# mika314/melonix

Hardware: AMD Instinct MI355X
Metric: STFT+pitch+resynth frames/sec (48 kHz, 4096 FFT, 256 hop); % HBM roofline (higher is better)
Workload: dtype f32

## Files before the change

melonix_amd/csrc/resynth_kernels.hip:

```cpp
#include <hip/hip_runtime.h>

#include "kernels.h"

#pragma clang fp contract(off)

namespace mx {

namespace {

constexpr int kResynthThreads = 128;

__global__ __launch_bounds__(kResynthThreads) void resynth_kernel(const ResynthArgs a) {
  const mx_step st = a.steps[blockIdx.x];
  const float *g = a.audio + MX_AUDIO_PAD + st.grain_start;
  const int L = st.grain_len;
  const float rate = st.rate;
  const float next = st.next_first;
  float *of = a.pcm_f32 ? a.pcm_f32 + st.out_offset : nullptr;
  int16_t *oi = a.pcm_i16 ? a.pcm_i16 + st.out_offset : nullptr;
  for (int i = threadIdx.x; i < st.sz; i += kResynthThreads) {
    const float x = (float)i * rate;
    const float ip = __builtin_truncf(x);
    const float f = x - ip;
    const int idx = (int)ip;
    const float a0 = g[idx];
    const float a1 = (idx + 1 < L) ? g[idx + 1] : next;
    const float v = (1.f - f) * a0 + f * a1;
    if (of) of[i] = v;
    if (oi) oi[i] = (int16_t)((double)v * 32767.);
  }
}

constexpr int kMaxGrain = 2304;

__device__ __forceinline__ float lerp_tap(const float *lg, int i, float rate) {
  const float x = (float)i * rate;
  const float ip = __builtin_truncf(x);
  const float f = x - ip;
  const int idx = (int)ip;
  return (1.f - f) * lg[idx] + f * lg[idx + 1];
}

__global__ __launch_bounds__(kResynthThreads) void resynth_kernel_v(const ResynthArgs a) {
  __shared__ __attribute__((aligned(16))) float lds[kMaxGrain + 8];
  const mx_step st = a.steps[blockIdx.x];
  const int L = st.grain_len, sz = st.sz, tid = threadIdx.x;
  const float *g = a.audio + MX_AUDIO_PAD + st.grain_start;
  if (L > kMaxGrain) {
    float *of = a.pcm_f32 ? a.pcm_f32 + st.out_offset : nullptr;
    int16_t *oi = a.pcm_i16 ? a.pcm_i16 + st.out_offset : nullptr;
    for (int i = tid; i < sz; i += kResynthThreads) {
      const float x = (float)i * st.rate;
      const float ip = __builtin_truncf(x);
      const float f = x - ip;
      const int idx = (int)ip;
      const float a1 = (idx + 1 < L) ? g[idx + 1] : st.next_first;
      const float v = (1.f - f) * g[idx] + f * a1;
      if (of) of[i] = v;
      if (oi) oi[i] = (int16_t)((double)v * 32767.);
    }
    return;
  }
  const int shift = (int)((reinterpret_cast<uintptr_t>(g) >> 2) & 3);
  const float4 *ga = reinterpret_cast<const float4 *>(g - shift);
  float4 *l4 = reinterpret_cast<float4 *>(lds);
  for (int j = tid; j < (L + shift + 4) / 4; j += kResynthThreads) l4[j] = ga[j];
  __syncthreads();
  float *lg = lds + shift;
  if (tid == 0) lg[L] = st.next_first;
  __syncthreads();

  float *of = a.pcm_f32 ? a.pcm_f32 + st.out_offset : nullptr;
  int16_t *oi = a.pcm_i16 ? a.pcm_i16 + st.out_offset : nullptr;
  const float rate = st.rate;
  const int head = (int)((8 - (st.out_offset & 7)) & 7) < sz ? (int)((8 - (st.out_offset & 7)) & 7) : sz;
  const int nv = (sz - head) / 8;
  for (int q = tid; q < nv; q += kResynthThreads) {
    const int i0 = head + 8 * q;
    float v[8];
#pragma unroll
    for (int k = 0; k < 8; ++k) v[k] = lerp_tap(lg, i0 + k, rate);
    if (of) {
      float4 *o4 = reinterpret_cast<float4 *>(of + i0);
      o4[0] = make_float4(v[0], v[1], v[2], v[3]);
      o4[1] = make_float4(v[4], v[5], v[6], v[7]);
    }
    if (oi) {
      unsigned w[4];
#pragma unroll
      for (int k = 0; k < 4; ++k) {
        const unsigned lo = (unsigned)(unsigned short)(int16_t)((double)v[2 * k] * 32767.);
        const unsigned hi = (unsigned)(unsigned short)(int16_t)((double)v[2 * k + 1] * 32767.);
        w[k] = lo | (hi << 16);
      }
      *reinterpret_cast<uint4 *>(oi + i0) = make_uint4(w[0], w[1], w[2], w[3]);
    }
  }
  const int tail0 = head + 8 * nv;
  for (int i = tid; i < head + (sz - tail0); i += kResynthThreads) {
    const int ii = i < head ? i : tail0 + (i - head);
    const float v = lerp_tap(lg, ii, rate);
    if (of) of[ii] = v;
    if (oi) oi[ii] = (int16_t)((double)v * 32767.);
  }
}

__device__ __forceinline__ uint64_t bit_range(int64_t base, int64_t lo, int64_t hi) {
  const int64_t s = lo - base > 0 ? lo - base : 0;
  const int64_t e = hi - base < 64 ? hi - base : 64;
  if (e <= s) return 0ull;
  const uint64_t upto_e = e >= 64 ? ~0ull : ((1ull << e) - 1ull);
  return upto_e & ~((1ull << s) - 1ull);
}

__global__ __launch_bounds__(256) void zc_kernel(const float *__restrict__ wav ,
                                                 int64_t n, uint64_t *__restrict__ zc7,
                                                 uint64_t *__restrict__ zc3) {
  const int lane = threadIdx.x & 63;
  const int64_t w0 = ((int64_t)blockIdx.x * 4 + (threadIdx.x >> 6)) * 64;
  const int64_t nwords = (n + 63) >> 6;
  if (w0 >= nwords) return;
  const float *p = wav + w0 * 64 + lane;
  const float xp = p[-64], xn = p[64 * 64];
  const uint64_t Aprev = __ballot(!(xp >= 0.f)), Bnext = __ballot(!(xn < 0.f));
  uint64_t A = 0, B = 0;
#pragma unroll 16
  for (int w = 0; w < 64; ++w) {
    const float x = p[64 * w];
    const uint64_t a = __ballot(!(x >= 0.f)), b = __ballot(!(x < 0.f));
    if (lane == w) {
      A = a;
      B = b;
    }
  }
  uint64_t Ap = ((uint64_t)(unsigned)__shfl_up((int)(A >> 32), 1) << 32) | (unsigned)__shfl_up((int)A, 1);
  uint64_t Bn = ((uint64_t)(unsigned)__shfl_down((int)(B >> 32), 1) << 32) | (unsigned)__shfl_down((int)B, 1);
  if (lane == 0) Ap = Aprev;
  if (lane == 63) Bn = Bnext;
  uint64_t ra3 = A, ra7 = A, rb3 = ~0ull, rb7 = ~0ull;
#pragma unroll
  for (int j = 1; j <= 7; ++j) {
    const uint64_t bj = (B >> j) | (Bn << (64 - j));
    rb7 &= bj;
    if (j <= 3) rb3 &= bj;
    if (j <= 6) {
      const uint64_t aj = (A << j) | (Ap >> (64 - j));
      ra7 &= aj;
      if (j <= 2) ra3 &= aj;
    }
  }
  const int64_t wi = w0 + lane;
  if (wi < nwords) {
    zc7[wi] = ra7 & rb7 & bit_range(wi * 64, 7, n - 7 - 1);
    zc3[wi] = ra3 & rb3 & bit_range(wi * 64, 3, n - 3 - 1);
  }
}

__global__ __launch_bounds__(256) void resynth_tail_kernel(const ResynthArgs a) {
  const mx_step last = a.steps[a.nsteps - 1];
  const int64_t covered = last.out_offset + (int64_t)last.sz;
  for (int64_t i = covered + (int64_t)blockIdx.x * 256 + threadIdx.x; i < a.nsamples; i += (int64_t)gridDim.x * 256) {
    if (a.pcm_f32) a.pcm_f32[i] = 0.f;
    if (a.pcm_i16) a.pcm_i16[i] = 0;
  }
}

}

hipError_t launch_resynth(const ResynthArgs &a, hipStream_t s) {
  if (a.nsteps > 0x7fffffffLL) return hipErrorInvalidValue;
  if (a.nsteps > 0) {
    hipLaunchKernelGGL(resynth_tail_kernel, dim3(64), dim3(256), 0, s, a);
    const bool aligned = ((reinterpret_cast<uintptr_t>(a.pcm_f32) | reinterpret_cast<uintptr_t>(a.pcm_i16) |
                           reinterpret_cast<uintptr_t>(a.audio)) & 15) == 0;
    if (aligned) {
      hipLaunchKernelGGL(resynth_kernel_v, dim3((unsigned)a.nsteps), dim3(kResynthThreads), 0, s, a);
    } else {
      hipLaunchKernelGGL(resynth_kernel, dim3((unsigned)a.nsteps), dim3(kResynthThreads), 0, s, a);
    }
    hipError_t e = hipGetLastError();
    if (e != hipSuccess) return e;
  }
  return hipSuccess;
}

hipError_t launch_zc_bitmaps(const float *audio_padded, int64_t n, uint64_t *zc7, uint64_t *zc3,
                             hipStream_t s) {
  if (n <= 0) return hipSuccess;
  const int64_t blocks = (((n + 63) >> 6) + 255) / 256;
  if (blocks > 0x7fffffffLL) return hipErrorInvalidValue;
  static_assert(MX_AUDIO_PAD >= 64 * 65, "zc_kernel reads one block row past either end of the audio");
  hipLaunchKernelGGL(zc_kernel, dim3((unsigned)blocks), dim3(256), 0, s, audio_padded + MX_AUDIO_PAD, n,
                     zc7, zc3);
  return hipGetLastError();
}

}
```

melonix_amd/csrc/stft_kernel_impl.h:

```cpp
#pragma once
#include <hip/hip_runtime.h>

#include "colormap_core.h"
#include "kernels.h"
#include "stft_core.h"
#include "stft_tables.h"

#define MX_BARRIER() __syncthreads()

namespace mx {

template <bool MAXOP>
__device__ __forceinline__ unsigned wave_reduce_u32(unsigned k) {
  constexpr unsigned ident = MAXOP ? 0u : 0xffffffffu;
#define MX_DPP_STEP(CTRL, ROWS)                                                                      \
  {                                                                                                  \
    const unsigned o = (unsigned)__builtin_amdgcn_update_dpp((int)ident, (int)k, CTRL, ROWS, 0xf, false); \
    k = MAXOP ? (o > k ? o : k) : (o < k ? o : k);                                                   \
  }
  MX_DPP_STEP(0xB1, 0xf)
  MX_DPP_STEP(0x4E, 0xf)
  MX_DPP_STEP(0x141, 0xf)
  MX_DPP_STEP(0x140, 0xf)
  MX_DPP_STEP(0x142, 0xa)
  MX_DPP_STEP(0x143, 0xc)
#undef MX_DPP_STEP
  return (unsigned)__builtin_amdgcn_readlane((int)k, 63);
}
__device__ __forceinline__ unsigned long long wave_max_u64(unsigned long long k) {
  const unsigned hi = (unsigned)(k >> 32), lo = (unsigned)k;
  const unsigned mhi = wave_reduce_u32<true>(hi);
  const unsigned long long tie = __ballot(hi == mhi);
  unsigned mlo;
  if (__builtin_popcountll(tie) == 1) mlo = (unsigned)__builtin_amdgcn_readlane((int)lo, __builtin_ctzll(tie));
  else mlo = wave_reduce_u32<true>(hi == mhi ? lo : 0u);
  return ((unsigned long long)mhi << 32) | mlo;
}

template <int IMM, bool NT = true>
__device__ __forceinline__ void st_row_nt(const float *base, unsigned off, float x) {
  static_assert(IMM >= -4096 && IMM <= 4095, "global_store immediate offset");
#if defined(__HIP_DEVICE_COMPILE__)
  if constexpr (NT) asm volatile("global_store_dword %0, %1, %2 offset:%3 nt" : : "v"(off), "v"(x), "s"(base), "n"(IMM) : "memory");
  else asm volatile("global_store_dword %0, %1, %2 offset:%3" : : "v"(off), "v"(x), "s"(base), "n"(IMM) : "memory");
#endif
}

template <class P, int MODE, int HOP, int WPE, bool DEFER = false, bool PREFETCH = false, bool CMAP = false, bool DIRECT = false,
          bool CIRC = false>
__global__ __launch_bounds__(P::T) __attribute__((amdgpu_waves_per_eu(WPE, WPE)))
void stft_kernel(const StftArgs a0) {
  const StftArgs &a = a0;
  using C = P;
  constexpr int N = P::N;
  constexpr int NW = C::T / 64;
  constexpr int kRed = (NW > 1) ? ((NW + 1) / 2) * 2 : 0;
  constexpr bool kTw3Bases = (P::R3 == 16);
  constexpr int kTw2 = ((C::TW2 + 1) / 2) * 2;
  static_assert(P::R3 == 16 || P::R3 == 8, "twiddle placement per plan");
  static_assert(!DIRECT || (NW > 1 && !DEFER && !CMAP), "direct row stores: multi-wave, non-deferred plans");
  static_assert(!CIRC || (MODE != kRanges && HOP == 0 && !PREFETCH && !CMAP), "circular window: bulk modes");
  constexpr int IMG = t1_size<C>();
  __shared__ __attribute__((aligned(16))) float2 lds[IMG + kRed + (DEFER ? C::M / 2 : 0) + kTw2];
  float *const lout = reinterpret_cast<float *>(DEFER ? lds + IMG + kRed : lds);
  float2 *const ltw2 = lds + IMG + kRed + (DEFER ? C::M / 2 : 0);

  const int t_ = threadIdx.x;
  const bool wave0 = __builtin_amdgcn_readfirstlane(t_) < 64;
  cpx u[kTw3Bases ? 1 : P::R3];
  cpx ulo;
  cpx w3r[kTw3Bases ? 1 : P::R3 - 1], w3base[6];
  if constexpr (kTw3Bases) {
    cpx uhi_unused;
    post_bases<P>(t_, a.ubase, ulo, uhi_unused);
    fetch_tw3_bases<P>(t_, a.tw3, w3base);
  } else {
    post_twiddles<P>(t_, a.ubase, *reinterpret_cast<cpx(*)[P::R3]>(&u));
    fetch_tw3<P>(t_, a.tw3, *reinterpret_cast<cpx(*)[P::R3 - 1]>(&w3r));
  }
  const uint32_t bmask_ = band_mask<P>(t_, a.kmin, a.kmax);
  uint32_t umask = 0;
#pragma unroll
  for (int o = 0; o < P::E; ++o) umask |= (__ballot((bmask_ >> o) & 1u) != 0ull) ? (1u << o) : 0u;
  umask = __builtin_amdgcn_readfirstlane(umask);
  constexpr bool kSlide = (MODE == kBulkAligned) && (HOP > 0) && Slide<P, (HOP > 0 ? HOP : 2)>::ok;
  constexpr int SD = Slide<P, (HOP > 0 ? HOP : 2)>::D;
  constexpr float kSc = 0.5f / (float)N;
  for (int i = t_; i < C::TW2; i += C::T) ltw2[i] = a.tw2[i];
  MX_BARRIER();

  unsigned lb = blockIdx.x;
  {
    const unsigned nb = gridDim.x, xcd = lb & 7u, q = nb >> 3, r = nb & 7u;
    lb = (xcd < r ? xcd * (q + 1) : r * (q + 1) + (xcd - r) * q) + (lb >> 3);
  }
  const int64_t f0 = (int64_t)lb * a.frames_per_block;
  const int64_t f1 = (f0 + a.frames_per_block < a.count) ? f0 + a.frames_per_block : a.count;

  cpx Y[P::E];
  cpx edge[SD], nx[SD];
  if constexpr (kSlide) {
    const int64_t e0 = (a.first_frame + f0 + 1) * (int64_t)HOP;
    if (f0 < f1) load_frame<P, 1, true>(t_, Y, a.audio + MX_AUDIO_PAD + (e0 - N), a.wtab);
    slide_edge<P, HOP>(t_, a.wtab, 2.0f * (float)N, edge);
  }

  unsigned long long *const red = reinterpret_cast<unsigned long long *>(lds + IMG);
  auto flush_pitch = [&](int64_t fr, int tt) {
    if (a.pitch && tt == 0) {
      unsigned long long b = red[0];
#pragma unroll
      for (int i = 1; i < NW; ++i) b = red[i] > b ? red[i] : b;
      mx_pitch p;
      p.bin = 0x7fffffff - (int)(unsigned)(b & 0xffffffffull);
      p.mag = __uint_as_float((unsigned)(b >> 32));
      a.pitch[fr] = p;
    }
  };
  const bool want_rows = a.mags != nullptr || (CMAP && a.rgb != nullptr);
  auto flush_row = [&](int64_t fr, int tt) {
    if (want_rows) {
      using f32x4 = float __attribute__((ext_vector_type(4)));
      const f32x4 *l4 = reinterpret_cast<const f32x4 *>(lout) + tt;
      f32x4 *row4 = reinterpret_cast<f32x4 *>(a.mags + (size_t)fr * (size_t)(N / 2)) + tt;
      f32x4 q[C::M / 4 / C::T];
#pragma unroll
      for (int i = 0; i < C::M / 4 / C::T; ++i) q[i] = l4[C::T * i];
      if (!CMAP || a.mags) {
#pragma unroll
        for (int i = 0; i < C::M / 4 / C::T; ++i) {
          __builtin_nontemporal_store(q[i], &row4[C::T * i]);
        }
      }
      if constexpr (CMAP) {
        if (a.rgb) {
          uint32_t *trow = reinterpret_cast<uint32_t *>(a.rgb + (size_t)fr * (size_t)(N / 2) * 3) + 3 * tt;
#pragma unroll 1
          for (int i = 0; i < C::M / 4 / C::T; ++i) {
            uint32_t w3[3];
            texel4(q[i].x, q[i].y, q[i].z, q[i].w, a.cmap_k, w3);
            uint32_t *o = trow + 3 * C::T * i;
            o[0] = w3[0];
            o[1] = w3[1];
            o[2] = w3[2];
          }
        }
      }
    }
  };

  auto frame_ptrs = [&](int64_t fr, int zo, const float *&x, const float *&w) {
    if constexpr (MODE == kRanges) {
      const int s = a.ranges[2 * fr], e = a.ranges[2 * fr + 1];
      const bool outside = (e <= 0) || ((int64_t)e - N >= a.n);
      x = outside ? a.audio : a.audio + MX_AUDIO_PAD + ((int64_t)e - N);
      int64_t d0 = (int64_t)N - ((int64_t)e - (int64_t)s);
      d0 = d0 < (int64_t)(N - 1 - kWOff) ? (int64_t)(N - 1 - kWOff) : d0;
      d0 = d0 > (int64_t)(kWDmax + kWTail) ? (int64_t)(kWDmax + kWTail) : d0;
      w = a.wext + kWOff + d0;
    } else {
      const int64_t e = (a.first_frame + fr + 1) * (int64_t)a.hop;
      x = a.audio + MX_AUDIO_PAD + (e - N);
      w = a.wtab + zo;
    }
  };
  float cpx_[2 * Circ<P>::CS], cpw_[2 * Circ<P>::CS];
  if constexpr (CIRC) {
    if (f0 < f1) {
      const int64_t pe = (a.first_frame + f0 + 1) * (int64_t)a.hop;
      circ_load_first<P>(t_, Y, a.audio + MX_AUDIO_PAD + (pe - N), a.wtab, circ_geo<P>(pe, a.hop).o);
    }
  }
  cpx xr[(PREFETCH && !kSlide) ? P::E : 1];
  if constexpr (PREFETCH && !kSlide) {
    if (f0 < f1) {
      const float *x0;
      const float *w0;
      frame_ptrs(f0, 0, x0, w0);
      load_raw<P, (MODE == kBulkAligned)>(t_, xr, x0);
    }
  }

  for (int64_t f = f0; f < f1; ++f) {
    int t = t_;
    unsigned bmask = bmask_;
    int zoff = 0;
    asm volatile("" : "+v"(t), "+v"(bmask), "+s"(zoff));
    int out_lo, out_hi;
    out_bases<P>(t, out_lo, out_hi);

    if constexpr (CIRC) {
      if (f > f0) {
        const int64_t pe = (a.first_frame + f + 1) * (int64_t)a.hop;
        const CircGeo<P> geo = circ_geo<P>(pe, a.hop);
        circ_fetch<P>(t, a.audio + MX_AUDIO_PAD + (pe - 2 * (int64_t)a.hop), a.wtab + zoff + (N - 2 * a.hop), geo, cpx_, cpw_);
        circ_step<P>(t, Y, a.decay, geo, cpx_, cpw_);
      }
    } else if constexpr (kSlide) {
      if (f > f0) slide_step<P, HOP>(Y, nx, edge, a.decay, kSc);
      if (f + 1 < f1) slide_fetch<P, HOP>(t, a.audio + MX_AUDIO_PAD + (a.first_frame + f + 2) * (int64_t)HOP, nx);
    } else {
      const float *x;
      const float *w;
      frame_ptrs(f, zoff, x, w);
      if constexpr (PREFETCH) {
        if constexpr (MODE == kRanges) apply_window<P, -1, false>(t, Y, xr, w);
        else apply_window_geo<P>(t, Y, xr, a.wtab + N + zoff, a.hop);
      } else if constexpr (MODE == kRanges) {
        load_frame<P, -1, false>(t, Y, x, w);
      } else {
        load_frame_geo<P, (MODE == kBulkAligned)>(t, Y, x, a.wtab + N + zoff, a.hop);
      }
    }

    cpx v[P::E];
    pass1<P>(Y, v);
    constexpr bool kTw2Batch = (P::NB2 == 1);
    store_t1<P>(t, v, lds);
    MX_BARRIER();
    if constexpr (DEFER || DIRECT) {
      if (f > f0) flush_pitch(f - 1, t);
    }
    if constexpr (kTw2Batch) {
      cpx w2[P::R2 - 1];
      load_t1_tw2<P>(t, v, lds, ltw2, w2);
      if constexpr (DEFER) {
        if (f > f0) flush_row(f - 1, t);
      }
      MX_BARRIER();
      pass2_reg<P>(v, w2);
    } else {
      load_t1<P>(t, v, lds);
      if constexpr (DEFER) {
        if (f > f0) flush_row(f - 1, t);
      }
      MX_BARRIER();
      pass2<P>(t, v, ltw2);
    }
    store_t2<P>(t, v, lds);
    MX_BARRIER();
    load_t2<P>(t, v, lds);
    MX_BARRIER();
    float mg[P::E];
    if (NW == 1 || wave0) {
      if constexpr (kTw3Bases) {
        pass3_bases<P, true>(t, v, w3base);
        post_fly<P, true>(t, v, ulo, csel(t == 0, mk(-1.0f, 0.0f), ulo), mg);
      } else {
        pass3_reg<P, true>(t, v, *reinterpret_cast<cpx(*)[P::R3 - 1]>(&w3r));
        post<P, true>(t, v, *reinterpret_cast<cpx(*)[P::R3]>(&u), mg);
      }
    } else {
      if constexpr (kTw3Bases) {
        pass3_bases<P, false>(t, v, w3base);
        post_fly<P, false>(t, v, ulo, ulo, mg);
      } else {
        pass3_reg<P, false>(t, v, *reinterpret_cast<cpx(*)[P::R3 - 1]>(&w3r));
        post<P, false>(t, v, *reinterpret_cast<cpx(*)[P::R3]>(&u), mg);
      }
    }

    if constexpr (PREFETCH && !kSlide) {
      if (f + 1 < f1) {
        const float *xn;
        const float *wn;
        frame_ptrs(f + 1, zoff, xn, wn);
        load_raw<P, (MODE == kBulkAligned)>(t, xr, xn);
      }
    }

    unsigned long long best = 0ull;
    if (a.pitch) {
      const unsigned klo = 0x7fffffffu - (unsigned)out_lo, khi = 0x7fffffffu - (unsigned)out_hi;
      const unsigned nlo = 0x7fffffffu - (unsigned)(C::M - out_lo), nhi = 0x7fffffffu - (unsigned)(C::M - out_hi);
#pragma unroll
      for (int s = 0; s < C::R3; ++s) {
        constexpr int H = C::R3 / 2;
        if (!((umask >> (2 * s)) & 3u)) continue;
        const unsigned b0 = (s < H ? klo : khi) - (unsigned)(C::NS3 * s);
        unsigned b1 = (s < H ? nlo : nhi) + (unsigned)(C::NS3 * s);
        if (s == H) b1 = (t == 0) ? 0x7fffffffu - (unsigned)(C::M / 2) : b1;
        const unsigned v0 = (unsigned)((int)(bmask << (31 - 2 * s)) >> 31);
        const unsigned v1 = (unsigned)((int)(bmask << (31 - (2 * s + 1))) >> 31);
        const unsigned long long k0 = ((unsigned long long)(__float_as_uint(mg[2 * s]) & v0) << 32) | (b0 & v0);
        const unsigned long long k1 = ((unsigned long long)(__float_as_uint(mg[2 * s + 1]) & v1) << 32) | (b1 & v1);
        best = k0 > best ? k0 : best;
        best = k1 > best ? k1 : best;
      }
      best = wave_max_u64(best);
      if constexpr (NW > 1) {
        if ((t & 63) == 0) red[t >> 6] = best;
      }
    }

    if constexpr (DIRECT) {
      if (want_rows) {
        const float *row = a.mags + (size_t)f * (size_t)(N / 2);
        constexpr int H = C::R3 / 2;
        constexpr int STEP = 4 * C::NS3;
        constexpr int G = 8192 / STEP;
        static_assert((STEP == 4096 || STEP == 2048) && H % G == 0, "slot groups share an offset through the store's immediate");
        const unsigned blo = 4u * (unsigned)out_lo, bhi = 4u * (unsigned)(out_hi + C::NS3 * H);
        const unsigned nlo = 4u * (unsigned)(C::M - out_lo), nhi = 4u * (unsigned)(C::M - out_hi - C::NS3 * H);
        static_for<0, C::R3>([&](auto ss) {
          constexpr int s = decltype(ss)::value;
          constexpr int sl = s < H ? s : s - H;
          constexpr int su = (sl & ~(G - 1)) + G / 2, sd = (sl & ~(G - 1)) + G / 2 - 1;
          const unsigned o0 = (s < H ? blo : bhi) + (unsigned)(su * STEP);
          unsigned o1 = (s < H ? nlo : nhi) - (unsigned)(sd * STEP);
          if constexpr (s == H) {
            o1 = (t == 0) ? (unsigned)(4 * (C::M / 2)) + (unsigned)((sl - sd) * STEP) : o1;
          }
          st_row_nt<(sl - su) * STEP>(row, o0, mg[2 * s]);
          st_row_nt<-(sl - sd) * STEP, false>(row, o1, mg[2 * s + 1]);
        });
      }
    } else if (want_rows) {
      float *plo = lout + out_lo, *phi = lout + out_hi;
      float *mlo = lout + (C::M - out_lo), *mhi = lout + (C::M - out_hi);
#pragma unroll
      for (int s = 0; s < C::R3; ++s) {
        constexpr int H = C::R3 / 2;
        (s < H ? plo : phi)[C::NS3 * s] = mg[2 * s];
        if (s == H) (t == 0 ? lout + C::M / 2 : mhi - C::NS3 * H)[0] = mg[2 * s + 1];
        else (s < H ? mlo : mhi)[-C::NS3 * s] = mg[2 * s + 1];
      }
    }
    if constexpr (!DEFER && !DIRECT) {
      if (want_rows) {
        MX_BARRIER();
        flush_row(f, t);
        MX_BARRIER();
      } else {
        MX_BARRIER();
      }
      if constexpr (NW > 1) {
        flush_pitch(f, t);
      } else if (a.pitch && t == 0) {
        mx_pitch p;
        p.bin = 0x7fffffff - (int)(unsigned)(best & 0xffffffffull);
        p.mag = __uint_as_float((unsigned)(best >> 32));
        a.pitch[f] = p;
      }
    }
  }
  if constexpr (DEFER || DIRECT) {
    if (f0 < f1) {
      MX_BARRIER();
      flush_pitch(f1 - 1, t_);
      if constexpr (DEFER) flush_row(f1 - 1, t_);
    }
  }
}


}
```

melonix_amd/csrc/stft_kernels.hip:

```cpp
#include <hip/hip_runtime.h>

#include "kernels.h"
#include "stft_kernel_impl.h"

namespace mx {

namespace {

template <class P>
struct Tune {
  static constexpr bool TWO_WAVE = (P::E == 16);
  static constexpr int WPE = TWO_WAVE ? 3 : 2;
  static constexpr bool PREFETCH = (P::E == 32);
  static constexpr bool slides(int hop) {
    return P::N == 4096 ? (hop == 256 || hop == 512) : P::N == 16384 ? (hop == 512 || hop == 1024) : hop == 1024;
  }
  static constexpr bool DIRECT = (P::N >= 16384);
  static constexpr bool CIRC = (P::N >= 16384);
  static constexpr bool DEFER = TWO_WAVE;
};

template <class P, int HOP>
bool try_slide(const StftArgs &b, dim3 grid, dim3 block, hipStream_t s) {
  if constexpr (Slide<P, HOP>::ok && Tune<P>::slides(HOP)) {
    if (b.hop != HOP) return false;
    hipLaunchKernelGGL((stft_kernel<P, kBulkAligned, HOP, Tune<P>::WPE, Tune<P>::DEFER, false, false, Tune<P>::DIRECT>),
                       grid, block, 0, s, b);
    return true;
  } else {
    return false;
  }
}

template <class P>
bool try_circ(const StftArgs &b, dim3 grid, dim3 block, hipStream_t s) {
  if constexpr (!Tune<P>::CIRC) {
    return false;
  } else {
    if (!Circ<P>::ok(b.hop)) return false;
    hipLaunchKernelGGL((stft_kernel<P, kBulkAny, 0, Tune<P>::WPE, Tune<P>::DEFER, false, false, Tune<P>::DIRECT, true>),
                       grid, block, 0, s, b);
    return true;
  }
}

template <class P>
hipError_t launch_plan(int mode, const StftArgs &a, hipStream_t s) {
  if (a.count <= 0) return hipSuccess;
  const int g = a.frames_per_block > 0 ? a.frames_per_block : 1;
  const int64_t blocks = (a.count + g - 1) / g;
  if (blocks > 0x7fffffffLL) return hipErrorInvalidValue;
  StftArgs b = a;
  b.frames_per_block = g;
  const dim3 grid((unsigned)blocks), block(P::T);
  constexpr int W = Tune<P>::WPE;
  constexpr bool DF = Tune<P>::DEFER, PF = Tune<P>::PREFETCH, DR = Tune<P>::DIRECT;
  switch (mode) {
    case kBulkAligned:
      if (!(try_slide<P, 256>(b, grid, block, s) || try_slide<P, 512>(b, grid, block, s) ||
            try_slide<P, 1024>(b, grid, block, s) || try_circ<P>(b, grid, block, s)))
        hipLaunchKernelGGL((stft_kernel<P, kBulkAligned, 0, W, DF, PF, false, DR>), grid, block, 0, s, b);
      break;
    case kBulkAny:
      if (try_circ<P>(b, grid, block, s)) break;
      hipLaunchKernelGGL((stft_kernel<P, kBulkAny, 0, W, DF, PF, false, DR>), grid, block, 0, s, b); break;
    case kRanges:
      if (a.rgb) hipLaunchKernelGGL((stft_kernel<P, kRanges, 0, (W > 2 ? 2 : W), DF, false, true>), grid, block, 0, s, b);
      else hipLaunchKernelGGL((stft_kernel<P, kRanges, 0, W, DF, false, false, DR>), grid, block, 0, s, b);
      break;
    default: return hipErrorInvalidValue;
  }
  return hipGetLastError();
}

}

int stft_points_per_thread(int N) { return N == 4096 ? kPlan4096E : 32; }

int stft_frames_per_block_cap(int N, int mode, int hop) {
  if (N == 32768 && mode != kRanges && Tune<Plan<32768, 32>>::CIRC && !Tune<Plan<32768, 32>>::slides(hop) &&
      Circ<Plan<32768, 32>>::ok(hop))
    return 32;
  return N == 32768 ? 8 : (N == 4096 ? 32 : 16);
}

hipError_t launch_stft(int N, int mode, const StftArgs &a, hipStream_t s) {
  switch (N) {
    case 4096: return launch_plan<Plan<4096, kPlan4096E>>(mode, a, s);
    case 16384: return launch_plan<Plan<16384, 32>>(mode, a, s);
    case 32768: return launch_plan<Plan<32768, 32>>(mode, a, s);
  }
  return hipErrorInvalidValue;
}

}
```

Baseline: 334.2 million.

## Fold resynth tail zeroing into main grid; pick pitch from row-flush registers

The separate tail-zeroing kernel is removed. Its work now runs in extra blocks appended to the resynth grid, which saves one launch. In the STFT kernel, a new ROWPICK variant computes the pitch argmax while the deferred two-wave row flush still holds the magnitudes in registers, replacing the band-mask ballot and the post-FFT argmax pass. When the band spans both waves, the partial maxima are combined through LDS with an extra barrier. This adds kernel variants and more template complexity.

```diff
diff --git a/melonix_amd/csrc/resynth_kernels.hip b/melonix_amd/csrc/resynth_kernels.hip
--- a/melonix_amd/csrc/resynth_kernels.hip
+++ b/melonix_amd/csrc/resynth_kernels.hip
@@ -10,7 +10,23 @@
 
 constexpr int kResynthThreads = 128;
 
+constexpr int kTailBlocks = 16;
+
+__device__ __forceinline__ void resynth_tail(const ResynthArgs &a, int tail_block) {
+  const mx_step last = a.steps[a.nsteps - 1];
+  const int64_t covered = last.out_offset + (int64_t)last.sz;
+  for (int64_t i = covered + (int64_t)tail_block * kResynthThreads + threadIdx.x; i < a.nsamples;
+       i += (int64_t)kTailBlocks * kResynthThreads) {
+    if (a.pcm_f32) a.pcm_f32[i] = 0.f;
+    if (a.pcm_i16) a.pcm_i16[i] = 0;
+  }
+}
+
 __global__ __launch_bounds__(kResynthThreads) void resynth_kernel(const ResynthArgs a) {
+  if (blockIdx.x >= a.nsteps) {
+    resynth_tail(a, (int)(blockIdx.x - a.nsteps));
+    __builtin_amdgcn_endpgm();
+  }
   const mx_step st = a.steps[blockIdx.x];
   const float *g = a.audio + MX_AUDIO_PAD + st.grain_start;
   const int L = st.grain_len;
@@ -43,6 +59,10 @@
 
 __global__ __launch_bounds__(kResynthThreads) void resynth_kernel_v(const ResynthArgs a) {
   __shared__ __attribute__((aligned(16))) float lds[kMaxGrain + 8];
+  if (blockIdx.x >= a.nsteps) {
+    resynth_tail(a, (int)(blockIdx.x - a.nsteps));
+    __builtin_amdgcn_endpgm();
+  }
   const mx_step st = a.steps[blockIdx.x];
   const int L = st.grain_len, sz = st.sz, tid = threadIdx.x;
   const float *g = a.audio + MX_AUDIO_PAD + st.grain_start;
@@ -156,27 +176,18 @@
   }
 }
 
-__global__ __launch_bounds__(256) void resynth_tail_kernel(const ResynthArgs a) {
-  const mx_step last = a.steps[a.nsteps - 1];
-  const int64_t covered = last.out_offset + (int64_t)last.sz;
-  for (int64_t i = covered + (int64_t)blockIdx.x * 256 + threadIdx.x; i < a.nsamples; i += (int64_t)gridDim.x * 256) {
-    if (a.pcm_f32) a.pcm_f32[i] = 0.f;
-    if (a.pcm_i16) a.pcm_i16[i] = 0;
-  }
-}
-
 }
 
 hipError_t launch_resynth(const ResynthArgs &a, hipStream_t s) {
-  if (a.nsteps > 0x7fffffffLL) return hipErrorInvalidValue;
+  if (a.nsteps > 0x7fffffffLL - kTailBlocks) return hipErrorInvalidValue;
   if (a.nsteps > 0) {
-    hipLaunchKernelGGL(resynth_tail_kernel, dim3(64), dim3(256), 0, s, a);
+    const dim3 grid((unsigned)a.nsteps + kTailBlocks);
     const bool aligned = ((reinterpret_cast<uintptr_t>(a.pcm_f32) | reinterpret_cast<uintptr_t>(a.pcm_i16) |
                            reinterpret_cast<uintptr_t>(a.audio)) & 15) == 0;
     if (aligned) {
-      hipLaunchKernelGGL(resynth_kernel_v, dim3((unsigned)a.nsteps), dim3(kResynthThreads), 0, s, a);
+      hipLaunchKernelGGL(resynth_kernel_v, grid, dim3(kResynthThreads), 0, s, a);
     } else {
-      hipLaunchKernelGGL(resynth_kernel, dim3((unsigned)a.nsteps), dim3(kResynthThreads), 0, s, a);
+      hipLaunchKernelGGL(resynth_kernel, grid, dim3(kResynthThreads), 0, s, a);
     }
     hipError_t e = hipGetLastError();
     if (e != hipSuccess) return e;
diff --git a/melonix_amd/csrc/stft_kernel_impl.h b/melonix_amd/csrc/stft_kernel_impl.h
--- a/melonix_amd/csrc/stft_kernel_impl.h
+++ b/melonix_amd/csrc/stft_kernel_impl.h
@@ -47,7 +47,7 @@
 }
 
 template <class P, int MODE, int HOP, int WPE, bool DEFER = false, bool PREFETCH = false, bool CMAP = false, bool DIRECT = false,
-          bool CIRC = false>
+          bool CIRC = false, bool ROWPICK = false>
 __global__ __launch_bounds__(P::T) __attribute__((amdgpu_waves_per_eu(WPE, WPE)))
 void stft_kernel(const StftArgs a0) {
   const StftArgs &a = a0;
@@ -60,6 +60,7 @@
   static_assert(P::R3 == 16 || P::R3 == 8, "twiddle placement per plan");
   static_assert(!DIRECT || (NW > 1 && !DEFER && !CMAP), "direct row stores: multi-wave, non-deferred plans");
   static_assert(!CIRC || (MODE != kRanges && HOP == 0 && !PREFETCH && !CMAP), "circular window: bulk modes");
+  static_assert(!ROWPICK || (DEFER && NW == 2), "row-side pick: the deferred two-wave row flush");
   constexpr int IMG = t1_size<C>();
   __shared__ __attribute__((aligned(16))) float2 lds[IMG + kRed + (DEFER ? C::M / 2 : 0) + kTw2];
   float *const lout = reinterpret_cast<float *>(DEFER ? lds + IMG + kRed : lds);
@@ -78,11 +79,28 @@
     post_twiddles<P>(t_, a.ubase, *reinterpret_cast<cpx(*)[P::R3]>(&u));
     fetch_tw3<P>(t_, a.tw3, *reinterpret_cast<cpx(*)[P::R3 - 1]>(&w3r));
   }
-  const uint32_t bmask_ = band_mask<P>(t_, a.kmin, a.kmax);
+  const uint32_t bmask_ = ROWPICK ? 0u : band_mask<P>(t_, a.kmin, a.kmax);
   uint32_t umask = 0;
-#pragma unroll
-  for (int o = 0; o < P::E; ++o) umask |= (__ballot((bmask_ >> o) & 1u) != 0ull) ? (1u << o) : 0u;
-  umask = __builtin_amdgcn_readfirstlane(umask);
+  if constexpr (!ROWPICK) {
+#pragma unroll
+    for (int o = 0; o < P::E; ++o) umask |= (__ballot((bmask_ >> o) & 1u) != 0ull) ? (1u << o) : 0u;
+    umask = __builtin_amdgcn_readfirstlane(umask);
+  }
+  constexpr int kChunks = C::M / 4 / C::T;
+  uint32_t cmask = 0;
+  bool pick_both = false;
+  if constexpr (ROWPICK) {
+    uint32_t cm[2] = {0u, 0u};
+#pragma unroll
+    for (int w = 0; w < 2; ++w)
+#pragma unroll
+      for (int i = 0; i < kChunks; ++i) {
+        const int lo = 4 * C::T * i + 256 * w;
+        cm[w] |= (a.kmin <= lo + 255 && a.kmax >= lo) ? (1u << i) : 0u;
+      }
+    cmask = wave0 ? cm[0] : cm[1];
+    pick_both = cm[0] != 0u && cm[1] != 0u;
+  }
   constexpr bool kSlide = (MODE == kBulkAligned) && (HOP > 0) && Slide<P, (HOP > 0 ? HOP : 2)>::ok;
   constexpr int SD = Slide<P, (HOP > 0 ? HOP : 2)>::D;
   constexpr float kSc = 0.5f / (float)N;
@@ -130,6 +148,36 @@
 #pragma unroll
         for (int i = 0; i < C::M / 4 / C::T; ++i) {
           __builtin_nontemporal_store(q[i], &row4[C::T * i]);
+        }
+      }
+      if constexpr (ROWPICK) {
+        if (a.pitch && cmask) {
+          const unsigned span = (unsigned)(a.kmax - a.kmin);
+          unsigned hi = 0u, lo = 0u;
+#pragma unroll
+          for (int i = kChunks - 1; i >= 0; --i) {
+            if (!((cmask >> i) & 1u)) continue;
+            const unsigned b0 = 4u * (unsigned)(tt + C::T * i);
+            const unsigned d0 = 4u * (unsigned)tt - (unsigned)a.kmin;
+#pragma unroll
+            for (int c = 3; c >= 0; --c) {
+              const unsigned m = __float_as_uint(q[i][c]);
+              const bool take = (d0 + (unsigned)(4 * C::T * i + c) <= span) && m >= hi;
+              hi = take ? m : hi;
+              lo = take ? 0x7fffffffu - (b0 + (unsigned)c) : lo;
+            }
+          }
+          const unsigned long long b = wave_max_u64(((unsigned long long)hi << 32) | lo);
+          if ((tt & 63) == 0) {
+            if (pick_both) {
+              red[tt >> 6] = b;
+            } else {
+              mx_pitch p;
+              p.bin = 0x7fffffff - (int)(unsigned)(b & 0xffffffffull);
+              p.mag = __uint_as_float((unsigned)(b >> 32));
+              a.pitch[fr] = p;
+            }
+          }
         }
       }
       if constexpr (CMAP) {
@@ -185,7 +233,8 @@
     int t = t_;
     unsigned bmask = bmask_;
     int zoff = 0;
-    asm volatile("" : "+v"(t), "+v"(bmask), "+s"(zoff));
+    if constexpr (ROWPICK) asm volatile("" : "+v"(t), "+s"(zoff));
+    else asm volatile("" : "+v"(t), "+v"(bmask), "+s"(zoff));
     int out_lo, out_hi;
     out_bases<P>(t, out_lo, out_hi);
 
@@ -218,7 +267,7 @@
     constexpr bool kTw2Batch = (P::NB2 == 1);
     store_t1<P>(t, v, lds);
     MX_BARRIER();
-    if constexpr (DEFER || DIRECT) {
+    if constexpr ((DEFER || DIRECT) && !ROWPICK) {
       if (f > f0) flush_pitch(f - 1, t);
     }
     if constexpr (kTw2Batch) {
@@ -228,6 +277,9 @@
         if (f > f0) flush_row(f - 1, t);
       }
       MX_BARRIER();
+      if constexpr (ROWPICK) {
+        if (pick_both && f > f0) flush_pitch(f - 1, t);
+      }
       pass2_reg<P>(v, w2);
     } else {
       load_t1<P>(t, v, lds);
@@ -235,6 +287,9 @@
         if (f > f0) flush_row(f - 1, t);
       }
       MX_BARRIER();
+      if constexpr (ROWPICK) {
+        if (pick_both && f > f0) flush_pitch(f - 1, t);
+      }
       pass2<P>(t, v, ltw2);
     }
     store_t2<P>(t, v, lds);
@@ -270,7 +325,7 @@
     }
 
     unsigned long long best = 0ull;
-    if (a.pitch) {
+    if (!ROWPICK && a.pitch) {
       const unsigned klo = 0x7fffffffu - (unsigned)out_lo, khi = 0x7fffffffu - (unsigned)out_hi;
       const unsigned nlo = 0x7fffffffu - (unsigned)(C::M - out_lo), nhi = 0x7fffffffu - (unsigned)(C::M - out_hi);
 #pragma unroll
@@ -347,8 +402,16 @@
   if constexpr (DEFER || DIRECT) {
     if (f0 < f1) {
       MX_BARRIER();
-      flush_pitch(f1 - 1, t_);
-      if constexpr (DEFER) flush_row(f1 - 1, t_);
+      if constexpr (ROWPICK) {
+        flush_row(f1 - 1, t_);
+        if (pick_both) {
+          MX_BARRIER();
+          flush_pitch(f1 - 1, t_);
+        }
+      } else {
+        flush_pitch(f1 - 1, t_);
+        if constexpr (DEFER) flush_row(f1 - 1, t_);
+      }
     }
   }
 }
diff --git a/melonix_amd/csrc/stft_kernels.hip b/melonix_amd/csrc/stft_kernels.hip
--- a/melonix_amd/csrc/stft_kernels.hip
+++ b/melonix_amd/csrc/stft_kernels.hip
@@ -20,12 +20,24 @@
   static constexpr bool DEFER = TWO_WAVE;
 };
 
+template <class P, int MODE, int HOP, int WPE, bool PREFETCH, bool CMAP, bool CIRC>
+void launch_kernel(const StftArgs &b, dim3 grid, dim3 block, hipStream_t s) {
+  constexpr bool DF = Tune<P>::DEFER, DR = !CMAP && Tune<P>::DIRECT;
+  if constexpr (DF) {
+    if (b.mags || (CMAP && b.rgb)) {
+      hipLaunchKernelGGL((stft_kernel<P, MODE, HOP, WPE, DF, PREFETCH, CMAP, DR, CIRC, true>), grid, block, 0, s, b);
+      return;
+    }
+  }
+  if constexpr (!(DF && CMAP))
+    hipLaunchKernelGGL((stft_kernel<P, MODE, HOP, WPE, DF, PREFETCH, CMAP, DR, CIRC, false>), grid, block, 0, s, b);
+}
+
 template <class P, int HOP>
 bool try_slide(const StftArgs &b, dim3 grid, dim3 block, hipStream_t s) {
   if constexpr (Slide<P, HOP>::ok && Tune<P>::slides(HOP)) {
     if (b.hop != HOP) return false;
-    hipLaunchKernelGGL((stft_kernel<P, kBulkAligned, HOP, Tune<P>::WPE, Tune<P>::DEFER, false, false, Tune<P>::DIRECT>),
-                       grid, block, 0, s, b);
+    launch_kernel<P, kBulkAligned, HOP, Tune<P>::WPE, false, false, false>(b, grid, block, s);
     return true;
   } else {
     return false;
@@ -38,8 +50,7 @@
     return false;
   } else {
     if (!Circ<P>::ok(b.hop)) return false;
-    hipLaunchKernelGGL((stft_kernel<P, kBulkAny, 0, Tune<P>::WPE, Tune<P>::DEFER, false, false, Tune<P>::DIRECT, true>),
-                       grid, block, 0, s, b);
+    launch_kernel<P, kBulkAny, 0, Tune<P>::WPE, false, false, true>(b, grid, block, s);
     return true;
   }
 }
@@ -54,19 +65,20 @@
   b.frames_per_block = g;
   const dim3 grid((unsigned)blocks), block(P::T);
   constexpr int W = Tune<P>::WPE;
-  constexpr bool DF = Tune<P>::DEFER, PF = Tune<P>::PREFETCH, DR = Tune<P>::DIRECT;
+  constexpr bool PF = Tune<P>::PREFETCH;
   switch (mode) {
     case kBulkAligned:
       if (!(try_slide<P, 256>(b, grid, block, s) || try_slide<P, 512>(b, grid, block, s) ||
             try_slide<P, 1024>(b, grid, block, s) || try_circ<P>(b, grid, block, s)))
-        hipLaunchKernelGGL((stft_kernel<P, kBulkAligned, 0, W, DF, PF, false, DR>), grid, block, 0, s, b);
+        launch_kernel<P, kBulkAligned, 0, W, PF, false, false>(b, grid, block, s);
       break;
     case kBulkAny:
       if (try_circ<P>(b, grid, block, s)) break;
-      hipLaunchKernelGGL((stft_kernel<P, kBulkAny, 0, W, DF, PF, false, DR>), grid, block, 0, s, b); break;
+      launch_kernel<P, kBulkAny, 0, W, PF, false, false>(b, grid, block, s);
+      break;
     case kRanges:
-      if (a.rgb) hipLaunchKernelGGL((stft_kernel<P, kRanges, 0, (W > 2 ? 2 : W), DF, false, true>), grid, block, 0, s, b);
-      else hipLaunchKernelGGL((stft_kernel<P, kRanges, 0, W, DF, false, false, DR>), grid, block, 0, s, b);
+      if (a.rgb) launch_kernel<P, kRanges, 0, (W > 2 ? 2 : W), false, true, false>(b, grid, block, s);
+      else launch_kernel<P, kRanges, 0, W, false, false, false>(b, grid, block, s);
       break;
     default: return hipErrorInvalidValue;
   }
```

Result: no change. 333.5 million (-0.2%).
